# AbrahamSanders/realtime-codec-agent

Hardware: AMD Instinct MI355X
Metric: batch-encode audio-hours/hour (+ xRT and p50 frame-step latency of 1 duplex stream in `duplex`) (higher is better)
Workload: dtype f32; 1 GPU; batch MagiCodec-style encode, 16 kHz stereo, 0.1 s chunks / 2.0 s context, 256 windows per step (BASELINE configs[1]); codebook=131072x16

## Files before the change

### include/rca.h

```cpp
#ifndef RCA_H
#define RCA_H

#include <stdint.h>

#ifdef __cplusplus
extern "C" {
#endif

#define RCA_OK 0
#define RCA_ERR_ARG -1
#define RCA_ERR_HIP -2
#define RCA_ERR_STATE -3
#define RCA_ERR_MISSING -4

#define RCA_MAX_STAGES 8

typedef struct rca_codec rca_codec_t;
typedef struct rca_lm rca_lm_t;

#define RCA_F32 0
#define RCA_BF16 1
#define RCA_Q8_0 2
#define RCA_F16 3
#define RCA_Q6_K 5
// ... 70 lines not shown
                              float* pcm_dev, void* stream);
int rca_codec_decode_rows_dev(rca_codec_t* h, const int64_t* codes_dev, const int64_t* src_off_dev, int32_t B, int32_t F, int32_t n_samples,
                              float* pcm_dev, const int64_t* dst_off_dev, int64_t code_span, int64_t pcm_span, void* stream);
int rca_codec_decode_error(rca_codec_t* h, void* stream, int32_t* raised);

#define RCA_JOIN_HEAD 1
#define RCA_JOIN_TAIL 2
typedef struct {
    int64_t seg_off;
    int64_t n;
    int64_t out_off;
    int32_t flags;
    int32_t reserved;
} rca_join_seg_t;
int rca_codec_crossfade_join_dev(rca_codec_t* h, const float* seg_dev, int64_t seg_span, const rca_join_seg_t* segs_dev,
                                 const rca_join_seg_t* segs_host, int32_t n_segs, const float* fade_in_dev, int32_t n_fade, float* out_dev,
                                 int64_t out_span, void* stream);

int rca_codec_encode_tail(rca_codec_t* h, const float* pcm_host, int32_t B, int32_t T, int32_t n_keep, int64_t* codes_host);
int rca_codec_decode_tail(rca_codec_t* h, const int64_t* codes_host, int32_t B, int32_t F, int32_t n_samples, float* pcm_host);
int rca_codec_set_stream_graphs(rca_codec_t* h, int32_t enable);
int rca_codec_set_mfma_mode(rca_codec_t* h, int32_t mode);
int rca_codec_receptive_field(const rca_codec_t* h, int32_t* enc_left_frames, int32_t* dec_left_frames);
int rca_codec_set_window_trim(rca_codec_t* h, int32_t enable);

int rca_codec_decode(rca_codec_t* h, const int64_t* codes_host, int32_t B, int32_t F, float* pcm_host);
int rca_codec_decode_dev(rca_codec_t* h, const int64_t* codes_dev, int32_t B, int32_t F, float* pcm_dev,
                         void* stream);

int rca_codec_encoder_dev(rca_codec_t* h, const float* pcm_dev, int32_t B, int32_t T, float* ze_dev, void* stream);
int rca_codec_quantize_dev(rca_codec_t* h, const float* ze_dev, int64_t rows, int64_t* codes_dev, void* stream);
int rca_codec_decoder_dev(rca_codec_t* h, const float* zq_dev, int32_t B, int32_t F, float* pcm_dev, void* stream);
int rca_codec_codebook_dev(rca_codec_t* h, const float** out_dev);

int rca_codec_codebook(rca_codec_t* h, float* out_host);

int rca_codec_encode_tap(rca_codec_t* h, const float* pcm_host, int32_t B, int32_t T, int32_t layer,
                         float* out_host, int64_t out_numel);

int rca_codec_encode_tap_bf16(rca_codec_t* h, const float* pcm_host, int32_t B, int32_t T, int32_t layer,
                              uint16_t* hi_host, uint16_t* lo_host, int64_t numel);

int rca_codec_set_variant(rca_codec_t* h, int32_t variant);

int rca_codec_profile(rca_codec_t* h, int32_t enable);
int rca_codec_profile_read(rca_codec_t* h, int32_t kclass, double* total_ms, int64_t* launches, double* flops,
// ... 127 lines not shown
```

### realtime_codec_agent_amd/_native.py

```python
from __future__ import annotations

import ctypes as C
import os
import subprocess
from typing import Dict, Iterable, List, Optional, Tuple

import numpy as np

_PKG_DIR = os.path.dirname(os.path.abspath(__file__))
CSRC_DIR = os.path.join(_PKG_DIR, "csrc")
LIB_PATH = os.environ.get("RCA_LIB_PATH") or os.path.join(_PKG_DIR, "librca_hip.so")
HIP_SOURCES = ["rca_codec.hip", "rca_lm.hip"]
HIPCC_FLAGS = ["--offload-arch=gfx950", "-O3", "-ffp-contract=off", "-std=c++17", "-fPIC", "-shared",
               "-Wno-unused-result", "-mllvm", "-amdgpu-kernarg-preload-count=14"]

MAX_STAGES = 8
RCA_F32, RCA_BF16, RCA_Q8_0, RCA_F16, RCA_Q4_K, RCA_Q6_K, RCA_Q5_K, RCA_Q4_0, RCA_Q4_1 = 0, 1, 2, 3, 4, 5, 6, 7, 8


class RcaError(RuntimeError):
    pass


class Q8Blocks:
# ... 306 lines not shown
            if verbose:
                print(" ".join(cmd))
            subprocess.check_call(cmd)
            os.replace(LIB_PATH + sfx, LIB_PATH)
            with open(_stamp_path() + sfx, "w") as f:
                f.write(key + "\n")
            os.replace(_stamp_path() + sfx, _stamp_path())
        finally:
            for t in tmps + [_stamp_path() + sfx]:
                if os.path.exists(t):
                    os.remove(t)
    return LIB_PATH


_lib = None

ABI_SYMBOLS = [
    "rca_last_error", "rca_device_count", "rca_device_sync", "rca_version",
    "rca_codec_create", "rca_codec_destroy", "rca_codec_hop", "rca_codec_num_frames",
    "rca_codec_encode", "rca_codec_encode_dev", "rca_codec_encode_windows_dev", "rca_codec_encode_chunk_range_dev", "rca_codec_encode_rows_dev",
    "rca_codec_ingest_rows_dev", "rca_codec_ingest_supported",
    "rca_codec_decode_rows_dev", "rca_codec_decode_error", "rca_codec_crossfade_join_dev",
    "rca_codec_decode", "rca_codec_decode_dev",
    "rca_codec_encode_tail_dev", "rca_codec_decode_tail_dev", "rca_codec_encode_tail", "rca_codec_decode_tail", "rca_codec_set_stream_graphs", "rca_codec_receptive_field", "rca_codec_set_window_trim",
    "rca_codec_encoder_dev", "rca_codec_quantize_dev", "rca_codec_decoder_dev", "rca_codec_codebook_dev",
    "rca_codec_codebook", "rca_codec_encode_tap", "rca_codec_encode_tap_bf16", "rca_codec_set_variant", "rca_codec_sync",
    "rca_codec_profile", "rca_codec_profile_read",
    "rca_lm_create", "rca_lm_create_random", "rca_lm_destroy", "rca_lm_reset", "rca_lm_eval",
    "rca_lm_get_n_tokens", "rca_lm_set_n_tokens", "rca_lm_get_logits", "rca_lm_get_logits_row",
    "rca_lm_logits_dev", "rca_lm_sampler_init", "rca_lm_sample", "rca_lm_step", "rca_lm_token_probs",
    "rca_lm_sync", "rca_lm_set_graphs", "rca_lm_mask_head_rows", "rca_lm_set_mfma_prefill", "rca_lm_set_logits_all",
    "rca_lm_persist_codec_embeddings", "rca_lm_create_shared", "rca_lm_eval_async", "rca_lm_copy_kv", "rca_lm_swap_kv",
    "rca_lm_set_low_priority", "rca_lm_frame", "rca_lm_weight_format", "rca_lm_set_attn_fuse", "rca_lm_prefill_route",
    "rca_lm_set_act_format", "rca_lm_get_act_format", "rca_lm_gemv_tap", "rca_lm_kv_remove", "rca_lm_kv_read",
    "rca_lm_kv_write", "rca_lm_attn_tap", "rca_lm_score", "rca_lm_score_rows_tap",
    "rca_duplex_frame", "rca_codec_workspace_sig", "rca_codec_stream_handoff", "rca_codec_codebook_size", "rca_codec_set_mfma_mode", "rca_lm_step_probe", "rca_duplex_prepare", "rca_duplex_precapture",
    "rca_lm_group_create", "rca_lm_group_destroy", "rca_lm_group_step",
]


def lib():
    global _lib
    if _lib is not None:
        return _lib
    if not os.path.exists(LIB_PATH):
        raise RcaError(
            f"{LIB_PATH} not found: build the HIP extension first (python -c 'import __graft_entry__ as g; g.build()'). "
# ... 55 lines not shown
```

### realtime_codec_agent_amd/codec.py

```python
from __future__ import annotations

import ctypes as C
from typing import Dict, Optional, Tuple

import numpy as np

from . import _native as N
from .codec_model import CodecConfig, init_codec_weights


class HipCodec:
    def __init__(self, cfg: CodecConfig, weights: Dict[str, np.ndarray], device: int = 0):
        self.cfg = cfg
        self.device = device
        self._lib = N.lib()
        self._h = C.c_void_p()
        tensors, keep = N.make_tensors(weights)
        ccfg = N.codec_config_c(cfg)
        N.check(self._lib.rca_codec_create(C.byref(ccfg), tensors, len(weights), device, C.byref(self._h)), "rca_codec_create")
        del keep
        self.hop = cfg.hop
        self.mfma_mode = 0

    def close(self):
# ... 102 lines not shown
                                                    C.c_void_p(lo.ctypes.data if lo is not None else None), C.c_int64(B * Cn * L)),
                "rca_codec_encode_tap_bf16")
        unblock = lambda a: np.ascontiguousarray(a.transpose(0, 1, 3, 2).reshape(B, Cn, L))
        return unblock(hi), (unblock(lo) if lo is not None else None)

    def encode_dev(self, pcm_ptr: int, B: int, T: int, codes_ptr: int, stream: int = 0) -> None:
        N.check(self._lib.rca_codec_encode_dev(self._h, C.c_void_p(pcm_ptr), B, T, C.c_void_p(codes_ptr), C.c_void_p(stream)), "rca_codec_encode_dev")

    def decode_dev(self, codes_ptr: int, B: int, F: int, pcm_ptr: int, stream: int = 0) -> None:
        N.check(self._lib.rca_codec_decode_dev(self._h, C.c_void_p(codes_ptr), B, F, C.c_void_p(pcm_ptr), C.c_void_p(stream)), "rca_codec_decode_dev")

    def encode_tail_dev(self, pcm_ptr: int, B: int, T: int, n_keep: int, codes_ptr: int, stream: int = 0) -> None:
        N.check(self._lib.rca_codec_encode_tail_dev(self._h, C.c_void_p(pcm_ptr), B, T, n_keep, C.c_void_p(codes_ptr), C.c_void_p(stream)),
                "rca_codec_encode_tail_dev")

    def decode_tail_dev(self, codes_ptr: int, B: int, F: int, n_samples: int, pcm_ptr: int, stream: int = 0) -> None:
        N.check(self._lib.rca_codec_decode_tail_dev(self._h, C.c_void_p(codes_ptr), B, F, n_samples, C.c_void_p(pcm_ptr), C.c_void_p(stream)),
                "rca_codec_decode_tail_dev")

    def receptive_field(self) -> Tuple[int, int]:
        a, b = C.c_int32(), C.c_int32()
        N.check(self._lib.rca_codec_receptive_field(self._h, C.byref(a), C.byref(b)), "rca_codec_receptive_field")
        return a.value, b.value

    def set_window_trim(self, enable: bool) -> None:
        N.check(self._lib.rca_codec_set_window_trim(self._h, int(bool(enable))), "rca_codec_set_window_trim")

    def encode_windows_dev(self, audio_ptr: int, Cn: int, Nsamp: int, chunk: int, ctx: int, batch_windows: int, codes_ptr: int,
                           codes_per_channel: int, stream: int = 0) -> None:
        N.check(self._lib.rca_codec_encode_windows_dev(self._h, C.c_void_p(audio_ptr), Cn, C.c_int64(Nsamp), chunk, ctx, batch_windows,
                                                       C.c_void_p(codes_ptr), C.c_int64(codes_per_channel), C.c_void_p(stream)),
                "rca_codec_encode_windows_dev")

    def encode_chunk_range_dev(self, audio_ptr: int, Cn: int, Nsamp: int, chunk: int, ctx: int, batch_windows: int, chunk_begin: int,
                               chunk_end: int, codes_ptr: int, codes_per_channel: int, stream: int = 0) -> None:
        N.check(self._lib.rca_codec_encode_chunk_range_dev(self._h, C.c_void_p(audio_ptr), Cn, C.c_int64(Nsamp), chunk, ctx, batch_windows,
                                                           C.c_int64(chunk_begin), C.c_int64(chunk_end), C.c_void_p(codes_ptr),
                                                           C.c_int64(codes_per_channel), C.c_void_p(stream)),
                "rca_codec_encode_chunk_range_dev")

    def encode_rows_dev(self, audio_ptr: int, src_off_ptr: int, B: int, T: int, n_keep: int, codes_ptr: int, dst_off_ptr: int, span: int,
                        stream: int = 0) -> None:
        N.check(self._lib.rca_codec_encode_rows_dev(self._h, C.c_void_p(audio_ptr), C.c_void_p(src_off_ptr), B, T, n_keep, C.c_void_p(codes_ptr),
                                                    C.c_void_p(dst_off_ptr), C.c_int64(span), C.c_void_p(stream)), "rca_codec_encode_rows_dev")

    def ingest_supported(self, up: int, down: int, n_taps: int) -> bool:
# ... 261 lines not shown
```

### realtime_codec_agent_amd/csrc/rca_codec.hip

```cpp
#include <stdarg.h>

#include <algorithm>
#include <array>
#include <cmath>
#include <map>
#include <type_traits>

#include "rca_common.h"

namespace rca {
thread_local char g_err[512] = {0};
}
using namespace rca;

typedef float f32x16 __attribute__((ext_vector_type(16)));

#define RCA_LAT_MAX_FRAMES 64
#define RCA_LDS_BUDGET (152 * 1024)

typedef float f32x4 __attribute__((ext_vector_type(4)));

struct RowSrc {
    const float* base;
    int C;
// ... 184 lines not shown
#ifndef RCA_CONV_WPB
#define RCA_CONV_WPB 1
#endif
#ifndef RCA_CONV_OCC
#define RCA_CONV_OCC 2
#endif
#ifndef RCA_CONV_PIPE
#define RCA_CONV_PIPE 1
#endif
#ifndef RCA_CONV_PRIO
#define RCA_CONV_PRIO 1
#endif
#ifndef RCA_CONV_ABUF
#define RCA_CONV_ABUF 1
#endif
#ifndef RCA_CONV_EPRIO
#define RCA_CONV_EPRIO 1
#endif
#ifdef RCA_ABL_NOBREAD
#define RCA_ABL_BREAD(x) (slope)
#else
#define RCA_ABL_BREAD(x) (x)
#endif
typedef __bf16 conv_bf16x8 __attribute__((ext_vector_type(8)));
typedef __bf16 conv_bf16x2 __attribute__((ext_vector_type(2)));
__device__ __forceinline__ unsigned conv_pack_bf16x2(float a, float b) {
    const conv_bf16x2 v = {(__bf16)a, (__bf16)b};
    return __builtin_bit_cast(unsigned, v);
}
template <int BF>
__device__ __forceinline__ void conv_split8(const float (&w)[8], uint4& hi, uint4& lo) {
    unsigned ph[4], pl[4];
#pragma unroll
    for (int j = 0; j < 4; ++j) {
        ph[j] = conv_pack_bf16x2(w[2 * j], w[2 * j + 1]);
        pl[j] = BF == 3 ? conv_pack_bf16x2(w[2 * j] - __uint_as_float(ph[j] << 16), w[2 * j + 1] - __uint_as_float(ph[j] & 0xffff0000u)) : 0u;
    }
    hi = make_uint4(ph[0], ph[1], ph[2], ph[3]);
    lo = make_uint4(pl[0], pl[1], pl[2], pl[3]);
}
template <int KS, int S, int CIC, int WM, int WN, int FUSE, int TR, int BF = 0, int FULLC = 0>
__global__ __launch_bounds__(64 * RCA_CONV_WPB, (((KS == 8 && CIC == 2) || (KS == 16 && CIC == 1)) && WM * WN < 8) ? 3 : RCA_CONV_OCC) void conv1d_mfma_kernel(const float* __restrict__ x, const float* __restrict__ wp,
                                                          const float* __restrict__ bias, float* __restrict__ y,
                                                          int Cin, int Lin, int Cout, int Lout, long Ncols, int nchunks,
                                                          int pre, float slope, FuseIn fin, TrInfo tr) {
    constexpr int MT = WM * 32;
// ... 191 lines not shown
        for (int q = 0; q < 4; ++q) {
            const f32x4 bq = *reinterpret_cast<const f32x4*>(bias + co0 + wm * 32 + 8 * q + 4 * half);
#pragma unroll
            for (int j = 0; j < 4; ++j)
#pragma unroll
                for (int wn = 0; wn < WN; ++wn) acc[wm][wn][4 * q + j] = bq[j];
        }
    }

    auto stage_write_t = [&](int buf, auto act_tag) __attribute__((always_inline)) {
        constexpr bool ACT = decltype(act_tag)::value;
#ifdef RCA_ABL_NOWRITE
        return;
#endif
        float* dst = xs + buf * BUF;
#pragma unroll
        for (int cl = 0; cl < CIC; ++cl) {
#pragma unroll
            for (int r = 0; r < RE; ++r) {
                float v[PW];
#pragma unroll
                for (int j = 0; j < PW; ++j) {
                    v[j] = sreg[cl][r][j];
                    if (ACT && !FUSE) v[j] = fmaxf(v[j], v[j] * slope);
                }
                if (U > NW + 2 || 64 * PW * (r + 1) <= E || s_loff[r] >= 0) {
#pragma unroll
                    for (int j = 0; j < PW; ++j) dst[cl * S * U + s_loff[r] + j * U] = v[j];
                }
            }
        }
    };
    auto stage_write = [&](int buf) __attribute__((always_inline)) {
        if (pre & 1) stage_write_t(buf, std::true_type{});
        else stage_write_t(buf, std::false_type{});
    };

    auto compute_t = [&](int buf, int cn, auto edge_tag) __attribute__((always_inline)) {
        constexpr bool EDGE = decltype(edge_tag)::value;
        const float* xb = xs + buf * BUF;
        const float4* pn[WM];
#pragma unroll
        for (int wm = 0; wm < WM; ++wm) pn[wm] = w_ptr(wm, cn);
        constexpr int NB = (KPC * WN > 32) ? ((KPC % 4 == 0) ? 4 : 2) : (KPC * WN == 32 && WN == 4) ? 2 : 1;
        constexpr int PB = KPC / NB;
        static_assert(KPC % NB == 0, "batching");
#pragma unroll
// ... 184 lines not shown
    }

    if (RCA_CONV_EPRIO) __builtin_amdgcn_s_setprio(0);
    RCA_TL_STAMP(tl2);
    const long orow = TR ? tr.Lout : Lout;
    const bool full_rows = co0 + MT <= Cout;
    float* const yw = y + ((long)b_base * Cout + co0) * orow;
#pragma unroll
    for (int wn = 0; wn < WN; ++wn) {
        const int dn = 1 - lead + wn * 32 + (lane & 31);
        if (dn >= ncol_left) continue;
        int bb, t;
        rel_bt(dn, bb, t);
        int ocol = t;
        if (TR) {
            ocol = tr.s * t - tr.padL + phase;
            if (ocol < 0 || ocol >= (int)orow) continue;
        }
        const unsigned voff = ((unsigned)bb * (unsigned)(Cout * (int)orow) + (unsigned)ocol + (unsigned)(4 * half) * (unsigned)orow) * 4u;
        if (pre & 2) {
#pragma unroll
            for (int wm = 0; wm < WM; ++wm)
#pragma unroll
                for (int r = 0; r < 16; ++r) acc[wm][wn][r] = fmaxf(acc[wm][wn][r], acc[wm][wn][r] * slope);
        }
        if (full_rows) {
#pragma unroll
            for (int wm = 0; wm < WM; ++wm)
#pragma unroll
                for (int r = 0; r < 16; ++r) {
                    const int cu = wm * 32 + (r & 3) + 8 * (r >> 2);
                    char* const yr = reinterpret_cast<char*>(yw + (long)cu * orow);
                    *reinterpret_cast<float*>(yr + voff) = acc[wm][wn][r];
                }
        } else {
#pragma unroll
            for (int wm = 0; wm < WM; ++wm)
#pragma unroll
                for (int r = 0; r < 16; ++r) {
                    const int cu = wm * 32 + (r & 3) + 8 * (r >> 2);
                    char* const yr = reinterpret_cast<char*>(yw + (long)cu * orow);
                    if (co0 + cu + 4 * half < Cout) *reinterpret_cast<float*>(yr + voff) = acc[wm][wn][r];
                }
        }
    }
#ifdef RCA_CONV_TIMELINE
    if (tl_buf && lane == 0) {
        const long tl3 = (long)wall_clock64();
        const unsigned hw = __builtin_amdgcn_s_getreg((31 << 11) | (0 << 6) | 4);
        const unsigned xcc = __builtin_amdgcn_s_getreg((3 << 11) | (0 << 6) | 20);
        constexpr int region = KS == 4 ? 0 : KS == 8 ? 1 : KS == 10 ? 2 : KS == 16 ? 3 : KS == 3 ? 4 : 5;
        long* o = tl_buf + ((long)region * 65536 + ((blockIdx.x * RCA_CONV_WPB + wave) & 0xFFFF)) * 8;
        o[6] = tl_load | (tl_mfma << 32);
        o[7] = tl_write | ((long)nchunks << 32);
        o[0] = tl0; o[1] = tl1; o[2] = tl2; o[3] = tl3;
        o[4] = (long)hw | ((long)xcc << 32);
        o[5] = (long)KS | ((long)S << 8) | ((long)WM << 16) | ((long)wave << 24) | ((long)blockIdx.x << 32);
    }
#endif
}

template <int NWN, bool PRE>
__global__ __launch_bounds__(64, 2) void conv_first_mfma_kernel(const float* __restrict__ wp, const float* __restrict__ bias,
                                                               float* __restrict__ y, int Cout, int Lout, long Ncols, int post, float slope,
                                                               FuseIn fin) {
    constexpr int NW = NWN * 32;
    constexpr int E = (NW + 2) * 2;
    constexpr int NBLK = 2 * NWN + 1;
    constexpr int RS = 136;
    constexpr int ZERO = 128;
    constexpr int CIN = 32, KQ = CIN / 2;
    extern __shared__ __attribute__((aligned(16))) float ring[];
#ifdef RCA_CONV_TIMELINE
    long* const tl_buf = rca_prof_buf;
#endif
    RCA_TL_STAMP(tl0);
    const int lane = threadIdx.x & 63;
    const int half = lane >> 5, jl = lane & 31;
    const int n_co = Cout / 64;
    const long wg = blockIdx.x;
    const int xcd = (int)(wg & 7);
    const long seq = wg >> 3;
    const int co_tile = __builtin_amdgcn_readfirstlane((int)(seq % n_co));
    const long n0 = ((seq / n_co) * 8 + xcd) * NW;
    const int co0 = co_tile * 64;
    if (n0 >= Ncols) return;
    const long n_base = n0 > 0 ? n0 - 1 : 0;
    const int b_base = __builtin_amdgcn_readfirstlane((int)((unsigned)n_base / (unsigned)Lout));
    const int t_base = (int)(n_base - (long)b_base * Lout);
    const int lead = n0 > 0 ? 0 : 1;
    const long left = Ncols - n_base;
    const int ncol_left = left > NW + 2 ? NW + 2 : (int)left;
    auto rel_bt = [&](int dn, int& bb, int& tt) {
        int dt = dn + t_base;
        bb = dt >= Lout ? 1 : 0;
        tt = bb ? dt - Lout : dt;
    };

    const int ch_in = jl;
    float a_in[4];
#pragma unroll
    for (int m = 0; m < 4; ++m) a_in[m] = (2 * m + half < 7) ? fin.w_in[ch_in * 7 + 2 * m + half] : -0.0f;
    f32x16 b_in;
#pragma unroll
    for (int r = 0; r < 16; ++r) b_in[r] = fin.b_in[(r & 3) + 8 * (r >> 2) + 4 * half];
    long o0, o1;
    if (fin.src.row_off) {
// ... 10 lines not shown
    const long om = o0 < o1 ? o0 : o1;
    const rca_rsrc_t rs_pcm = rca_make_rsrc(fin.src.base + om, 0x7FFFFFFF);
    const unsigned prow0 = (unsigned)(o0 - om), prow1 = (unsigned)(o1 - om);
    constexpr unsigned OOB = 0x80000000u;
    auto pcm_load = [&](int bk, float (&pb)[4]) __attribute__((always_inline)) {
        const int e = 32 * bk + jl;
        const int dn = (e >> 1) - lead;
        const bool ok = e < E && dn >= 0 && dn < ncol_left;
        int bb, t;
        rel_bt(ok ? dn : 0, bb, t);
        const int i = 2 * t + (e & 1) - 3 + half;
        const unsigned ro = bb ? prow1 : prow0;
#pragma unroll
        for (int m = 0; m < 4; ++m) {
            const int j = i + 2 * m;
            const unsigned off = (ok && 2 * m + half < 7 && j >= 0 && j < fin.src.T) ? (ro + (unsigned)j) * 4u : OOB;
            pb[m] = rca_buffer_load_f32(rs_pcm, (int)off, 0, 0);
        }
    };
    auto cin_mfma = [&](int m, const float (&pb)[4], f32x16& d) __attribute__((always_inline)) {
        d = __builtin_amdgcn_mfma_f32_32x32x2f32(a_in[m], pb[m], m == 0 ? b_in : d, 0, 0, 0);
    };
    const int w_lane = 4 * half * RS + jl;
    auto cin_write = [&](int bk, f32x16& d, int r0, int r1) __attribute__((always_inline)) {
#pragma unroll
        for (int r = r0; r < r1; ++r) {
            float v = d[r];
            if (PRE) v = fmaxf(v, v * slope);
            ring[w_lane + ((r & 3) + 8 * (r >> 2)) * RS + ((32 * bk) & 127)] = v;
        }
    };

    if (lane < CIN) ring[lane * RS + ZERO] = 0.0f;
    float pa[4], pb[4];
    float4 a[2][KQ];
    {
        float p2[4];
        pcm_load(0, pa);
        pcm_load(1, pb);
        pcm_load(2, p2);
        __builtin_amdgcn_sched_barrier(0);
        const rca_rsrc_t rs_w = rca_make_rsrc(reinterpret_cast<const float4*>(wp) + (long)co_tile * 2 * KQ * 64, 0x7FFFFFFF);
#pragma unroll
        for (int wm = 0; wm < 2; ++wm)
#pragma unroll
            for (int q = 0; q < KQ; ++q) {
                const rca_f32x4_t v = rca_buffer_load_f32x4(rs_w, lane * 16, (wm * KQ + q) * 1024, 0);
                a[wm][q] = make_float4(v[0], v[1], v[2], v[3]);
            }
        __builtin_amdgcn_sched_barrier(0);
        f32x16 d0, d1;
#pragma unroll
        for (int m = 0; m < 4; ++m) { cin_mfma(m, pa, d0); cin_mfma(m, pb, d1); }
        cin_write(0, d0, 0, 16);
#pragma unroll
        for (int m = 0; m < 4; ++m) cin_mfma(m, p2, d0);
        cin_write(1, d1, 0, 16);
        cin_write(2, d0, 0, 16);
    }
    if (NBLK > 3) pcm_load(3, pa);
    if (NBLK > 4) pcm_load(4, pb);
    __builtin_amdgcn_wave_barrier();
    RCA_TL_STAMP(tl1);
#ifdef RCA_CONV_TIMELINE
    long tl_load = 1 << 30, tl_mfma = 0, tl_write = 0;
#endif

    const rca_rsrc_t rs_y = rca_make_rsrc(y + ((long)b_base * Cout + co0) * Lout, 0x7FFFFFFF);
    __builtin_amdgcn_s_setprio(RCA_CONV_EPRIO);
#pragma unroll
    for (int wn = 0; wn < NWN; ++wn) {
        RCA_TL_STAMP(ta);
        const int j = 32 * wn + jl;
        int bz, tz;
        rel_bt(1 - lead + j, bz, tz);
        const int ad0 = (half == 0 && tz == 0) ? ZERO : ((2 * j + 1 + half) & 127);
        const int ad1 = (half == 1 && tz == Lout - 1) ? ZERO : ((2 * j + 3 + half) & 127);
        f32x16 acc[2];
#pragma unroll
        for (int wm = 0; wm < 2; ++wm)
#pragma unroll
            for (int q = 0; q < 4; ++q) {
                const f32x4 bq = *reinterpret_cast<const f32x4*>(bias + co0 + wm * 32 + 8 * q + 4 * half);
#pragma unroll
                for (int jj = 0; jj < 4; ++jj) acc[wm][4 * q + jj] = bq[jj];
            }
        const bool more = 2 * wn + 4 < NBLK;
        f32x16 d;
        float bcur[4], bnxt[4];
        auto b_read = [&](int c, float (&bv)[4]) __attribute__((always_inline)) {
#pragma unroll
            for (int cl = 0; cl < 2; ++cl) {
                bv[2 * cl] = ring[ad0 + (2 * c + cl) * RS];
                bv[2 * cl + 1] = ring[ad1 + (2 * c + cl) * RS];
            }
        };
        b_read(0, bcur);
#pragma unroll
        for (int c = 0; c < KQ; ++c) {
            if (c + 1 < KQ) b_read(c + 1, bnxt);
#pragma unroll
            for (int kp = 0; kp < 4; ++kp) {
#pragma unroll
                for (int wm = 0; wm < 2; ++wm) {
                    const float4 q4 = a[wm][c];
                    const float av = kp == 0 ? q4.x : kp == 1 ? q4.y : kp == 2 ? q4.z : q4.w;
                    acc[wm] = __builtin_amdgcn_mfma_f32_32x32x2f32(av, bcur[kp], acc[wm], 0, 0, 0);
                }
                if (c == 0 && 2 * wn + 3 < NBLK) cin_mfma(kp, pa, d);
                if (c == 3 && more) cin_mfma(kp, pb, d);
            }
            if (c == 2 && 2 * wn + 3 < NBLK) cin_write(2 * wn + 3, d, 0, 16);
            if (more && c >= 4 && (c & 3) == 3) cin_write(2 * wn + 4, d, 4 * (c >> 2) - 4, 4 * (c >> 2));
            if (c == 1 && 2 * wn + 5 < NBLK) pcm_load(2 * wn + 5, pa);
            if (c == 4 && 2 * wn + 6 < NBLK) pcm_load(2 * wn + 6, pb);
            if (c + 1 < KQ) {
#pragma unroll
                for (int i = 0; i < 4; ++i) bcur[i] = bnxt[i];
            }
            __builtin_amdgcn_sched_barrier(0);
        }
        if (more) cin_write(2 * wn + 4, d, 12, 16);
        __builtin_amdgcn_wave_barrier();
        RCA_TL_STAMP(tb);
        const int dn = 1 - lead + j;
        int bb, t;
        rel_bt(dn, bb, t);
        const unsigned voff = dn < ncol_left ? ((unsigned)bb * (unsigned)(Cout * Lout) + (unsigned)t + (unsigned)(4 * half * Lout)) * 4u : OOB;
        if (post) {
#pragma unroll
            for (int wm = 0; wm < 2; ++wm)
#pragma unroll
                for (int r = 0; r < 16; ++r) acc[wm][r] = fmaxf(acc[wm][r], acc[wm][r] * slope);
        }
#pragma unroll
        for (int wm = 0; wm < 2; ++wm)
#pragma unroll
            for (int r = 0; r < 16; ++r) rca_buffer_store_f32(acc[wm][r], rs_y, (int)voff, (wm * 32 + (r & 3) + 8 * (r >> 2)) * Lout * 4, 0);
        RCA_TL_STAMP(tc);
        RCA_TL_MIN(tl_load, ta, tb); RCA_TL_ADD(tl_mfma, ta, tb); RCA_TL_ADD(tl_write, tb, tc);
    }
    if (RCA_CONV_EPRIO) __builtin_amdgcn_s_setprio(0);
    RCA_TL_STAMP(tl2);
#ifdef RCA_CONV_TIMELINE
    if (tl_buf && lane == 0) {
        const long tl3 = (long)wall_clock64();
        const unsigned hw = __builtin_amdgcn_s_getreg((31 << 11) | (0 << 6) | 4);
        const unsigned xcc = __builtin_amdgcn_s_getreg((3 << 11) | (0 << 6) | 20);
        long* o = tl_buf + ((long)blockIdx.x & 0xFFFF) * 8;
        o[6] = tl_load | (tl_mfma << 32);
        o[7] = tl_write | ((long)(2 * NWN) << 32);
        o[0] = tl0; o[1] = tl1; o[2] = tl2; o[3] = tl3;
        o[4] = (long)hw | ((long)xcc << 32);
        o[5] = 4L | (2L << 8) | (2L << 16) | ((long)blockIdx.x << 32);
    }
#endif
}

template <int KS, int S, int CIC, int FUSE>
__global__ __launch_bounds__(512) void conv1d_ws_kernel(const float* __restrict__ x, const float* __restrict__ wp,
                                                        const float* __restrict__ bias, float* __restrict__ y,
                                                        int Cin, int Lin, int Cout, int Lout, long Ncols, int nchunks,
                                                        int pre, float slope, FuseIn fin) {
    constexpr int WM = 2, WN = 2;
    constexpr int MT = WM * 32, NW = WN * 32;
    constexpr int U = ConvLds<S>::stride(NW);
    constexpr int KPC = CIC * KS / 2;
    constexpr int QPC = KPC / 4;
    constexpr int E = (NW + 2) * S;
    constexpr int RE = (E + 63) / 64;
    constexpr int padL = (KS - S + 1) / 2;
    constexpr int BUF = CIC * S * U + 4;
    constexpr int WBUF = WM * QPC * 64 * 4;
    static_assert(KPC % 4 == 0 && KPC <= 64, "chunk shape");
// ... 1369 lines not shown
    if (!h) return fail(RCA_ERR_ARG, "null");
    RCA_HIP(hipSetDevice(h->device));
    RCA_HIP(hipStreamSynchronize(h->stream));
    return RCA_OK;
}

template <int KS, int S, int CIC, int WM, int WN, int FUSE, int TR, int BF = 0>
static void launch_conv_cfg(const ConvLayer& L, const float* wp, int nchunks, const float* x, float* y, int Lin, int Lc, long Ncols,
                            float slope, const FuseIn& fin, const TrInfo& tr, hipStream_t st, int act) {
    constexpr int NT = RCA_CONV_WPB * WN * 32, MT = WM * 32;
    constexpr int lds = RCA_CONV_WPB * 2 * (CIC * S * ConvLds<S>::stride(WN * 32) + 4) * 4;
    static_assert(lds <= 65536, "LDS budget");
    const long col_tiles = (cdiv(Ncols, NT) + 7) / 8 * 8;
    dim3 grid((unsigned)(col_tiles * cdiv(L.cout, MT) * (TR ? tr.s : 1)));
    if constexpr (!FUSE && !TR && BF == 0) {
        if (L.cin % CIC == 0 && nchunks * CIC == L.cin) {
            conv1d_mfma_kernel<KS, S, CIC, WM, WN, 0, 0, 0, 1><<<grid, 64 * RCA_CONV_WPB, lds, st>>>(x, wp, L.bp, y, L.cin, Lin, L.cout, Lc, Ncols, nchunks, act, slope, fin, tr);
            return;
        }
    }
    conv1d_mfma_kernel<KS, S, CIC, WM, WN, FUSE, TR, BF><<<grid, 64 * RCA_CONV_WPB, lds, st>>>(x, wp, L.bp, y, L.cin, Lin, L.cout, Lc, Ncols, nchunks, act, slope, fin, tr);
}

template <int KS, int S, int CIC>
static int launch_conv_mfma(const ConvLayer& L, const float* x, float* y, int B, int Lin, int Lout, float slope, hipStream_t st,
                            const FuseIn* fuse = nullptr, int act = -1, int bf = 0) {
    if (act < 0) act = L.pre;
    const long Ncols = (long)B * Lout;
    if (bf) {
        const FuseIn none_b{};
        const TrInfo notr_b{};
        const bool big = (long)cdiv(Ncols, 64) * cdiv(L.cout, 64) >= 2048;
#define RCA_BF_LAUNCH(FU, BFM) do { \
            if (big) launch_conv_cfg<KS, S, CIC, 2, 2, FU, 0, BFM>(L, L.wp, L.nchunks, x, y, Lin, Lout, Ncols, slope, FU ? *fuse : none_b, notr_b, st, act); \
            else launch_conv_cfg<KS, S, CIC, 1, 1, FU, 0, BFM>(L, L.wp, L.nchunks, x, y, Lin, Lout, Ncols, slope, FU ? *fuse : none_b, notr_b, st, act); } while (0)
        if constexpr (KS == 4 || KS == 8 || KS == 16) {
            if (fuse) { if (bf == 3) RCA_BF_LAUNCH(1, 3); else RCA_BF_LAUNCH(1, 1); RCA_LAUNCH_CHECK(); return RCA_OK; }
        }
        if (fuse) return fail(RCA_ERR_ARG, "internal: fused first layer of this shape has no bf16 instantiation");
        if (bf == 3) RCA_BF_LAUNCH(0, 3); else RCA_BF_LAUNCH(0, 1);
#undef RCA_BF_LAUNCH
        RCA_LAUNCH_CHECK();
        return RCA_OK;
    }
    const long waves_big = (long)cdiv(Ncols, 64) * cdiv(L.cout, 64);
#ifdef RCA_CONV_FORCE_MID
    constexpr long BIG_MIN = 1L << 40, MID_MIN = 2048;
#else
    constexpr long BIG_MIN = 8192, MID_MIN = 2048;
#endif
    const FuseIn none{};
    const TrInfo notr{};
    if (fuse) {
        static const bool wide = []() { const char* e = getenv("RCA_FUSE_WIDE"); return !(e && e[0] == '0'); }();
        if constexpr (KS == 4 && S == 2) {
            const char* mi = getenv("RCA_FUSE_MFMA_IN");
            constexpr int NWN = 4;
            if (!(mi && mi[0] == '0') && wide && waves_big >= BIG_MIN && Lout >= NWN * 32 + 3 && L.cin == 32 && L.cout % 64 == 0) {
                const long col_tiles = (cdiv(Ncols, NWN * 32) + 7) / 8 * 8;
                const dim3 grid((unsigned)(col_tiles * (L.cout / 64)));
                constexpr int lds = 32 * 136 * 4;
                if (act & 1) conv_first_mfma_kernel<NWN, true><<<grid, 64, lds, st>>>(L.wp, L.bp, y, L.cout, Lout, Ncols, act & 2, slope, *fuse);
                else conv_first_mfma_kernel<NWN, false><<<grid, 64, lds, st>>>(L.wp, L.bp, y, L.cout, Lout, Ncols, act & 2, slope, *fuse);
                RCA_LAUNCH_CHECK();
                return RCA_OK;
            }
            if (wide && waves_big >= BIG_MIN && Lout >= 131 && L.cin % 2 == 0) {
                launch_conv_cfg<4, 2, 2, 2, 4, 1, 0>(L, L.wp, L.cin / 2, x, y, Lin, Lout, Ncols, slope, *fuse, notr, st, act);
                RCA_LAUNCH_CHECK();
                return RCA_OK;
            }
        }
        if (waves_big >= BIG_MIN) launch_conv_cfg<KS, S, CIC, 2, 2, 1, 0>(L, L.wp, L.nchunks, x, y, Lin, Lout, Ncols, slope, *fuse, notr, st, act);
        else launch_conv_cfg<KS, S, CIC, 1, 1, 1, 0>(L, L.wp, L.nchunks, x, y, Lin, Lout, Ncols, slope, *fuse, notr, st, act);
    } else {
        if (waves_big >= BIG_MIN) launch_conv_cfg<KS, S, CIC, 2, 2, 0, 0>(L, L.wp, L.nchunks, x, y, Lin, Lout, Ncols, slope, none, notr, st, act);
        else if (waves_big >= MID_MIN) launch_conv_cfg<KS, S, CIC, 1, 2, 0, 0>(L, L.wp, L.nchunks, x, y, Lin, Lout, Ncols, slope, none, notr, st, act);
        else if (KS == 3 && L.cout >= 64 && waves_big >= 1024) launch_conv_cfg<KS, S, CIC, (KS == 3 ? 2 : 1), 1, 0, 0>(L, L.wp, L.nchunks, x, y, Lin, Lout, Ncols, slope, none, notr, st, act);
        else launch_conv_cfg<KS, S, CIC, 1, 1, 0, 0>(L, L.wp, L.nchunks, x, y, Lin, Lout, Ncols, slope, none, notr, st, act);
    }
    RCA_LAUNCH_CHECK();
    return RCA_OK;
}

static int launch_convtr_mfma(const ConvLayer& L, const float* x, float* y, int B, int Lin, float slope, hipStream_t st) {
    const int Lc = Lin + 1;
// ... 282 lines not shown
                         esz * (double)Ly.cin * Ly.k * Ly.cout);
        const Bf16Pack& wp = h->bf16_packs[li];
        const conv_bf16raw *xh = hi_of(cur), *xl = lo_of(cur);
        conv_bf16raw *yh = hi_of(cur ^ 1), *yl = lo_of(cur ^ 1);
        float* yf = h->act[cur ^ 1].as<float>();
        if (!split && Ly.k == 10 && Ly.cout % 256 == 0) rc = launch_conv_bf16<10, 5, 4, 1, 0, 0, 2>(split, Ly, wp, xh, xl, yh, yl, yf, B, L, act, slope, st);
        else if (last) rc = launch_conv_bf16<3, 1, 4, 4, 1>(split, Ly, wp, xh, xl, yh, yl, yf, B, L, act, slope, st);
        else if (Ly.k == 4 && li == 1 && fuse_in)
            rc = launch_conv_bf16<4, 2, 2, 2, 0, 1>(split, Ly, wp, xh, xl, yh, yl, yf, B, L, act, slope, st, src, h->bf16_packs[0].w_in8, Ly.pre ? 1 : 0);
        else if (Ly.k == 4) rc = launch_conv_bf16<4, 2, 2, 2, 0>(split, Ly, wp, xh, xl, yh, yl, yf, B, L, act, slope, st);
        else if (Ly.k == 8) rc = launch_conv_bf16<8, 4, 4, 1, 0>(split, Ly, wp, xh, xl, yh, yl, yf, B, L, act, slope, st);
        else if (Ly.k == 10) rc = launch_conv_bf16<10, 5, 4, 1, 0>(split, Ly, wp, xh, xl, yh, yl, yf, B, L, act, slope, st);
        else rc = launch_conv_bf16<16, 8, 4, 1, 0>(split, Ly, wp, xh, xl, yh, yl, yf, B, L, act, slope, st);
        if (rc != RCA_OK) return rc;
        L = Lout;
        cur ^= 1;
        if (last && tap_layer == (int)li) RCA_HIP(hipMemcpyAsync(tap_dev, yf, (size_t)B * Ly.cout * L * 4, hipMemcpyDeviceToDevice, st));
        if (stop_at((int)li)) return RCA_OK;
    }
    *ze_out = h->act[cur].as<float>();
    return RCA_OK;
}

static int run_encoder(rca_codec* h, RowSrc src, int B, hipStream_t st, float** ze_out, int* F_out, int tap_layer, float* tap_dev,
                       int bf16_tap = -1, const conv_bf16raw** bf16_planes = nullptr, int keep = 0, int* Fz_out = nullptr) {
    const rca_codec_config_t& c = h->cfg;
    const int F = (src.T + h->hop - 1) / h->hop;
    const int Tp = F * h->hop;
    if (F < 1) return fail(RCA_ERR_ARG, "empty audio (T=%d)", src.T);
    if (Fz_out) *Fz_out = F;
    size_t max_elems = 0;
    {
        long L = Tp;
        max_elems = std::max(max_elems, (size_t)B * c.channels[0] * L);
        for (int i = 0; i < c.n_stages; ++i) { L /= c.strides[i]; max_elems = std::max(max_elems, (size_t)B * c.channels[i + 1] * L); }
        max_elems = std::max(max_elems, (size_t)B * c.latent_dim * L);
    }
    int rc;
    if ((rc = h->act[0].ensure(max_elems * 4)) != RCA_OK) return rc;
    if ((rc = h->act[1].ensure(max_elems * 4)) != RCA_OK) return rc;
    if (bf16_blk_ok(h, tap_layer) && (double)B * max_elems < 4.0e18 && Tp / h->enc[1].s >= 64) {
        *F_out = F;
        return run_encoder_bf16(h, src, B, Tp, max_elems, st, ze_out, tap_layer, tap_dev, bf16_tap, bf16_planes);
    }
    if (bf16_tap >= 0) return fail(RCA_ERR_ARG, "bf16 tap: encode() does not take the blocked bf16 pipeline here (mfma mode %d, B=%d T=%d)", h->mfma_mode, B, src.T);
    int cur = 0;
    int L = Tp;
    size_t first = 1;
    const ConvLayer& E0 = h->enc[0];
    const ConvLayer& E1 = h->enc[1];
    const bool fuse01 = !h->lat_mode && h->variant >= 1 && tap_layer != 0 && E0.k == 7 && E1.wp && E1.k == 2 * E1.s && (double)B * E1.cin * L < 4.0e9 &&
                        ((E1.k == 4 && E1.s == 2) || (E1.k == 8 && E1.s == 4) || (E1.k == 16 && E1.s == 8)) && L / E1.s >= 67 &&
                        (double)E1.cout * (L / E1.s) < 2.6e8 &&
                        (src.row_off ? (double)src.span : (double)src.C * (double)std::labs(src.chan_stride) + (double)std::labs(src.win_stride) + src.T) < 5.0e8;
    bool prev_post = false;
    auto handoff = [&](size_t next, int Lnext) {
        return tap_layer < 0 && h->variant == 1 && !h->lat_mode && next < h->enc.size() && h->enc[next].pre && mfma_conv_ok(h, h->enc[next], B, Lnext, 0);
    };
    if (fuse01) {
        float* y = h->act[cur].as<float>();
        FuseIn fin{src, E0.w, E0.b};
        const float slope = c.leaky_slope;
        const int Lout = L / E1.s;
        {
            ProfScope ps(h, st, 0, 2.0 * E1.cin * E1.k * E1.cout * (double)B * Lout + 2.0 * E0.k * E0.cout * (double)B * L,
                         4.0 * ((double)B * src.T + (double)B * E1.cout * Lout + (double)E1.cin * E1.k * E1.cout));
            prev_post = handoff(2, Lout);
            const int act = (E1.pre ? 1 : 0) | (prev_post ? 2 : 0);
            if (h->variant == 2 && try_conv_ws(E1, nullptr, y, B, L, Lout, slope, st, &fin)) { rc = RCA_OK; RCA_LAUNCH_CHECK(); }
            else if (E1.k == 4) rc = launch_conv_mfma<4, 2, 4>(E1, nullptr, y, B, L, Lout, slope, st, &fin, act, h->mfma_mode);
            else if (E1.k == 8) rc = launch_conv_mfma<8, 4, RCA_CIC_K8>(E1, nullptr, y, B, L, Lout, slope, st, &fin, act, h->mfma_mode);
            else rc = launch_conv_mfma<16, 8, RCA_CIC_K16>(E1, nullptr, y, B, L, Lout, slope, st, &fin, act, h->mfma_mode);
        }
        if (rc != RCA_OK) return rc;
        L = Lout;
        first = 2;
// ... 102 lines not shown
    RowDst dst{codes, B, (long)F, 0, F};
    return run_quantize(h, ze, 0, B, F, 0, F, dst, st, nullptr);
}

static int trimmable_frames(const rca_codec* h, int F, int keep) { return std::max(0, F - keep - h->enc_left_frames); }

extern "C" int rca_codec_encode_tail_dev(rca_codec_t* h, const float* pcm, int32_t B, int32_t T, int32_t n_keep, int64_t* codes,
                                         void* stream) {
    if (!h || !pcm || !codes || B < 1 || T < 1 || n_keep < 1) return fail(RCA_ERR_ARG, "encode_tail: bad argument (B=%d T=%d keep=%d)", B, T, n_keep);
    const int F = (T + h->hop - 1) / h->hop;
    if (n_keep > F) return fail(RCA_ERR_ARG, "encode_tail: %d frames wanted, the window holds %d", n_keep, F);
    RCA_HIP(hipSetDevice(h->device));
    hipStream_t st = pick_stream(h, stream);
    const int j = trimmable_frames(h, F, n_keep);
    RowSrc src{pcm + (long)j * h->hop, B, (long)T, 0, T - j * h->hop};
    float* ze; int Ft, rc;
    h->lat_mode = h->variant >= 1 && (long)B * (F - j) <= RCA_LAT_MAX_FRAMES;
    int Fz;
    rc = run_encoder(h, src, B, st, &ze, &Ft, -1, nullptr, -1, nullptr, n_keep, &Fz);
    h->lat_mode = false;
    if (rc != RCA_OK) return rc;
    RowDst dst{codes, B, (long)n_keep, 0, n_keep};
    return run_quantize(h, ze, 0, B, Fz, Fz - n_keep, n_keep, dst, st, nullptr);
}

extern "C" int rca_codec_receptive_field(const rca_codec_t* h, int32_t* enc_left_frames, int32_t* dec_left_frames) {
    if (!h || !enc_left_frames || !dec_left_frames) return fail(RCA_ERR_ARG, "null");
    *enc_left_frames = h->enc_left_frames;
    *dec_left_frames = h->dec_left_frames;
    return RCA_OK;
}

extern "C" int rca_codec_set_window_trim(rca_codec_t* h, int32_t enable) {
    if (!h) return fail(RCA_ERR_ARG, "null");
    h->window_trim = enable != 0;
    return RCA_OK;
}

extern "C" int rca_codec_encode(rca_codec_t* h, const float* pcm_host, int32_t B, int32_t T, int64_t* codes_host) {
    if (!h || !pcm_host || !codes_host || B < 1 || T < 1) return fail(RCA_ERR_ARG, "encode: bad argument (B=%d T=%d)", B, T);
    RCA_HIP(hipSetDevice(h->device));
    const int F = (T + h->hop - 1) / h->hop;
    int rc;
    if ((rc = h->io_a.ensure((size_t)B * T * 4)) != RCA_OK) return rc;
    if ((rc = h->io_b.ensure((size_t)B * F * 8)) != RCA_OK) return rc;
    RCA_HIP(hipMemcpyAsync(h->io_a.p, pcm_host, (size_t)B * T * 4, hipMemcpyHostToDevice, h->stream));
// ... 634 lines not shown
```

Baseline: 3496 audio-hours/hour.

## Choose first-layer fused conv column width per shape, with runtime group count

The fused first conv MFMA kernel used to process a fixed 4 groups of 32 columns per wave. It can now take a runtime group count picked by a cost model over slots, so each wave covers more columns and amortizes the ring prologue and epilogue. The loop is restructured into even and odd parity groups so ring offsets stay compile-time. Leaky ReLU now uses an inline v_max_f32 asm helper, and a plan-query API is added. The risks are fewer waves, which lowers occupancy and parallelism, and weaker unrolling in the runtime-count path.

```diff
diff --git a/include/rca.h b/include/rca.h
--- a/include/rca.h
+++ b/include/rca.h
@@ -116,6 +116,7 @@
 int rca_codec_set_stream_graphs(rca_codec_t* h, int32_t enable);
 int rca_codec_set_mfma_mode(rca_codec_t* h, int32_t mode);
 int rca_codec_receptive_field(const rca_codec_t* h, int32_t* enc_left_frames, int32_t* dec_left_frames);
+int rca_codec_first_layer_plan(const rca_codec_t* h, int32_t B, int32_t T, int32_t* cols_per_wave);
 int rca_codec_set_window_trim(rca_codec_t* h, int32_t enable);
 
 int rca_codec_decode(rca_codec_t* h, const int64_t* codes_host, int32_t B, int32_t F, float* pcm_host);
diff --git a/realtime_codec_agent_amd/_native.py b/realtime_codec_agent_amd/_native.py
--- a/realtime_codec_agent_amd/_native.py
+++ b/realtime_codec_agent_amd/_native.py
@@ -352,7 +352,7 @@
     "rca_codec_ingest_rows_dev", "rca_codec_ingest_supported",
     "rca_codec_decode_rows_dev", "rca_codec_decode_error", "rca_codec_crossfade_join_dev",
     "rca_codec_decode", "rca_codec_decode_dev",
-    "rca_codec_encode_tail_dev", "rca_codec_decode_tail_dev", "rca_codec_encode_tail", "rca_codec_decode_tail", "rca_codec_set_stream_graphs", "rca_codec_receptive_field", "rca_codec_set_window_trim",
+    "rca_codec_encode_tail_dev", "rca_codec_decode_tail_dev", "rca_codec_encode_tail", "rca_codec_decode_tail", "rca_codec_set_stream_graphs", "rca_codec_receptive_field", "rca_codec_first_layer_plan", "rca_codec_set_window_trim",
     "rca_codec_encoder_dev", "rca_codec_quantize_dev", "rca_codec_decoder_dev", "rca_codec_codebook_dev",
     "rca_codec_codebook", "rca_codec_encode_tap", "rca_codec_encode_tap_bf16", "rca_codec_set_variant", "rca_codec_sync",
     "rca_codec_profile", "rca_codec_profile_read",
diff --git a/realtime_codec_agent_amd/codec.py b/realtime_codec_agent_amd/codec.py
--- a/realtime_codec_agent_amd/codec.py
+++ b/realtime_codec_agent_amd/codec.py
@@ -148,6 +148,11 @@
         a, b = C.c_int32(), C.c_int32()
         N.check(self._lib.rca_codec_receptive_field(self._h, C.byref(a), C.byref(b)), "rca_codec_receptive_field")
         return a.value, b.value
+
+    def first_layer_plan(self, B: int, T: int) -> int:
+        n = C.c_int32()
+        N.check(self._lib.rca_codec_first_layer_plan(self._h, int(B), int(T), C.byref(n)), "rca_codec_first_layer_plan")
+        return n.value
 
     def set_window_trim(self, enable: bool) -> None:
         N.check(self._lib.rca_codec_set_window_trim(self._h, int(bool(enable))), "rca_codec_set_window_trim")
diff --git a/realtime_codec_agent_amd/csrc/rca_codec.hip b/realtime_codec_agent_amd/csrc/rca_codec.hip
--- a/realtime_codec_agent_amd/csrc/rca_codec.hip
+++ b/realtime_codec_agent_amd/csrc/rca_codec.hip
@@ -230,6 +230,12 @@
 #else
 #define RCA_ABL_BREAD(x) (x)
 #endif
+__device__ __forceinline__ float conv_lrelu(float v, float slope) {
+    const float m = v * slope;
+    float r;
+    asm("v_max_f32 %0, %1, %2" : "=v"(r) : "v"(v), "v"(m));
+    return r;
+}
 typedef __bf16 conv_bf16x8 __attribute__((ext_vector_type(8)));
 typedef __bf16 conv_bf16x2 __attribute__((ext_vector_type(2)));
 __device__ __forceinline__ unsigned conv_pack_bf16x2(float a, float b) {
@@ -467,7 +473,7 @@
 #pragma unroll
                 for (int j = 0; j < PW; ++j) {
                     v[j] = sreg[cl][r][j];
-                    if (ACT && !FUSE) v[j] = fmaxf(v[j], v[j] * slope);
+                    if (ACT && !FUSE) v[j] = conv_lrelu(v[j], slope);
                 }
                 if (U > NW + 2 || 64 * PW * (r + 1) <= E || s_loff[r] >= 0) {
 #pragma unroll
@@ -698,7 +704,7 @@
 #pragma unroll
             for (int wm = 0; wm < WM; ++wm)
 #pragma unroll
-                for (int r = 0; r < 16; ++r) acc[wm][wn][r] = fmaxf(acc[wm][wn][r], acc[wm][wn][r] * slope);
+                for (int r = 0; r < 16; ++r) acc[wm][wn][r] = conv_lrelu(acc[wm][wn][r], slope);
         }
         if (full_rows) {
 #pragma unroll
@@ -739,10 +745,11 @@
 template <int NWN, bool PRE>
 __global__ __launch_bounds__(64, 2) void conv_first_mfma_kernel(const float* __restrict__ wp, const float* __restrict__ bias,
                                                                float* __restrict__ y, int Cout, int Lout, long Ncols, int post, float slope,
-                                                               FuseIn fin) {
-    constexpr int NW = NWN * 32;
-    constexpr int E = (NW + 2) * 2;
-    constexpr int NBLK = 2 * NWN + 1;
+                                                               FuseIn fin, int ngroups) {
+    static_assert(NWN % 2 == 0, "a wave walks whole ring periods");
+    const int ng = NWN ? NWN : ngroups;
+    const int NW = ng * 32;
+    const int E = (NW + 2) * 2;
     constexpr int RS = 136;
     constexpr int ZERO = 128;
     constexpr int CIN = 32, KQ = CIN / 2;
@@ -758,7 +765,7 @@
     const int xcd = (int)(wg & 7);
     const long seq = wg >> 3;
     const int co_tile = __builtin_amdgcn_readfirstlane((int)(seq % n_co));
-    const long n0 = ((seq / n_co) * 8 + xcd) * NW;
+    const long n0 = ((seq / n_co) * 8 + xcd) * (long)NW;
     const int co0 = co_tile * 64;
     if (n0 >= Ncols) return;
     const long n_base = n0 > 0 ? n0 - 1 : 0;
@@ -815,12 +822,12 @@
         d = __builtin_amdgcn_mfma_f32_32x32x2f32(a_in[m], pb[m], m == 0 ? b_in : d, 0, 0, 0);
     };
     const int w_lane = 4 * half * RS + jl;
-    auto cin_write = [&](int bk, f32x16& d, int r0, int r1) __attribute__((always_inline)) {
+    auto cin_write = [&](int rb, f32x16& d, int r0, int r1) __attribute__((always_inline)) {
 #pragma unroll
         for (int r = r0; r < r1; ++r) {
             float v = d[r];
-            if (PRE) v = fmaxf(v, v * slope);
-            ring[w_lane + ((r & 3) + 8 * (r >> 2)) * RS + ((32 * bk) & 127)] = v;
+            if (PRE) v = conv_lrelu(v, slope);
+            ring[w_lane + ((r & 3) + 8 * (r >> 2)) * RS + rb] = v;
         }
     };
 
@@ -848,11 +855,11 @@
         cin_write(0, d0, 0, 16);
 #pragma unroll
         for (int m = 0; m < 4; ++m) cin_mfma(m, p2, d0);
-        cin_write(1, d1, 0, 16);
-        cin_write(2, d0, 0, 16);
-    }
-    if (NBLK > 3) pcm_load(3, pa);
-    if (NBLK > 4) pcm_load(4, pb);
+        cin_write(32, d1, 0, 16);
+        cin_write(64, d0, 0, 16);
+    }
+    pcm_load(3, pa);
+    pcm_load(4, pb);
     __builtin_amdgcn_wave_barrier();
     RCA_TL_STAMP(tl1);
 #ifdef RCA_CONV_TIMELINE
@@ -861,24 +868,26 @@
 
     const rca_rsrc_t rs_y = rca_make_rsrc(y + ((long)b_base * Cout + co0) * Lout, 0x7FFFFFFF);
     __builtin_amdgcn_s_setprio(RCA_CONV_EPRIO);
-#pragma unroll
-    for (int wn = 0; wn < NWN; ++wn) {
+    auto group = [&](auto par_tag, auto cin_tag, auto pcm_tag, int wn) __attribute__((always_inline)) {
+        constexpr int PAR = decltype(par_tag)::value;
+        constexpr bool CIN = decltype(cin_tag)::value, PCM = decltype(pcm_tag)::value;
         RCA_TL_STAMP(ta);
         const int j = 32 * wn + jl;
         int bz, tz;
         rel_bt(1 - lead + j, bz, tz);
-        const int ad0 = (half == 0 && tz == 0) ? ZERO : ((2 * j + 1 + half) & 127);
-        const int ad1 = (half == 1 && tz == Lout - 1) ? ZERO : ((2 * j + 3 + half) & 127);
+        const int ad0 = (half == 0 && tz == 0) ? ZERO : ((64 * PAR + 2 * jl + 1 + half) & 127);
+        const int ad1 = (half == 1 && tz == Lout - 1) ? ZERO : ((64 * PAR + 2 * jl + 3 + half) & 127);
         f32x16 acc[2];
+        int bias_o = co0;
+        if (NWN == 0) asm volatile("" : "+s"(bias_o));
 #pragma unroll
         for (int wm = 0; wm < 2; ++wm)
 #pragma unroll
             for (int q = 0; q < 4; ++q) {
-                const f32x4 bq = *reinterpret_cast<const f32x4*>(bias + co0 + wm * 32 + 8 * q + 4 * half);
+                const f32x4 bq = *reinterpret_cast<const f32x4*>(bias + bias_o + wm * 32 + 8 * q + 4 * half);
 #pragma unroll
                 for (int jj = 0; jj < 4; ++jj) acc[wm][4 * q + jj] = bq[jj];
             }
-        const bool more = 2 * wn + 4 < NBLK;
         f32x16 d;
         float bcur[4], bnxt[4];
         auto b_read = [&](int c, float (&bv)[4]) __attribute__((always_inline)) {
@@ -900,20 +909,20 @@
                     const float av = kp == 0 ? q4.x : kp == 1 ? q4.y : kp == 2 ? q4.z : q4.w;
                     acc[wm] = __builtin_amdgcn_mfma_f32_32x32x2f32(av, bcur[kp], acc[wm], 0, 0, 0);
                 }
-                if (c == 0 && 2 * wn + 3 < NBLK) cin_mfma(kp, pa, d);
-                if (c == 3 && more) cin_mfma(kp, pb, d);
-            }
-            if (c == 2 && 2 * wn + 3 < NBLK) cin_write(2 * wn + 3, d, 0, 16);
-            if (more && c >= 4 && (c & 3) == 3) cin_write(2 * wn + 4, d, 4 * (c >> 2) - 4, 4 * (c >> 2));
-            if (c == 1 && 2 * wn + 5 < NBLK) pcm_load(2 * wn + 5, pa);
-            if (c == 4 && 2 * wn + 6 < NBLK) pcm_load(2 * wn + 6, pb);
+                if (c == 0 && CIN) cin_mfma(kp, pa, d);
+                if (c == 3 && CIN) cin_mfma(kp, pb, d);
+            }
+            if (c == 2 && CIN) cin_write((64 * PAR + 96) & 127, d, 0, 16);
+            if (CIN && c >= 4 && (c & 3) == 3) cin_write(64 * PAR, d, 4 * (c >> 2) - 4, 4 * (c >> 2));
+            if (c == 1 && PCM) pcm_load(2 * wn + 5, pa);
+            if (c == 4 && PCM) pcm_load(2 * wn + 6, pb);
             if (c + 1 < KQ) {
 #pragma unroll
                 for (int i = 0; i < 4; ++i) bcur[i] = bnxt[i];
             }
             __builtin_amdgcn_sched_barrier(0);
         }
-        if (more) cin_write(2 * wn + 4, d, 12, 16);
+        if (CIN) cin_write(64 * PAR, d, 12, 16);
         __builtin_amdgcn_wave_barrier();
         RCA_TL_STAMP(tb);
         const int dn = 1 - lead + j;
@@ -924,7 +933,7 @@
 #pragma unroll
             for (int wm = 0; wm < 2; ++wm)
 #pragma unroll
-                for (int r = 0; r < 16; ++r) acc[wm][r] = fmaxf(acc[wm][r], acc[wm][r] * slope);
+                for (int r = 0; r < 16; ++r) acc[wm][r] = conv_lrelu(acc[wm][r], slope);
         }
 #pragma unroll
         for (int wm = 0; wm < 2; ++wm)
@@ -932,7 +941,17 @@
             for (int r = 0; r < 16; ++r) rca_buffer_store_f32(acc[wm][r], rs_y, (int)voff, (wm * 32 + (r & 3) + 8 * (r >> 2)) * Lout * 4, 0);
         RCA_TL_STAMP(tc);
         RCA_TL_MIN(tl_load, ta, tb); RCA_TL_ADD(tl_mfma, ta, tb); RCA_TL_ADD(tl_write, tb, tc);
-    }
+    };
+    constexpr std::integral_constant<int, 0> even{};
+    constexpr std::integral_constant<int, 1> odd{};
+    constexpr int UNROLL = NWN ? NWN / 2 : 1;
+#pragma unroll UNROLL
+    for (int wn = 0; wn < ng - 2; wn += 2) {
+        group(even, std::true_type{}, std::true_type{}, wn);
+        group(odd, std::true_type{}, std::true_type{}, wn + 1);
+    }
+    group(even, std::true_type{}, std::false_type{}, ng - 2);
+    group(odd, std::false_type{}, std::false_type{}, ng - 1);
     if (RCA_CONV_EPRIO) __builtin_amdgcn_s_setprio(0);
     RCA_TL_STAMP(tl2);
 #ifdef RCA_CONV_TIMELINE
@@ -942,7 +961,7 @@
         const unsigned xcc = __builtin_amdgcn_s_getreg((3 << 11) | (0 << 6) | 20);
         long* o = tl_buf + ((long)blockIdx.x & 0xFFFF) * 8;
         o[6] = tl_load | (tl_mfma << 32);
-        o[7] = tl_write | ((long)(2 * NWN) << 32);
+        o[7] = tl_write | ((long)(2 * ng) << 32);
         o[0] = tl0; o[1] = tl1; o[2] = tl2; o[3] = tl3;
         o[4] = (long)hw | ((long)xcc << 32);
         o[5] = 4L | (2L << 8) | (2L << 16) | ((long)blockIdx.x << 32);
@@ -2358,6 +2377,27 @@
     conv1d_mfma_kernel<KS, S, CIC, WM, WN, FUSE, TR, BF><<<grid, 64 * RCA_CONV_WPB, lds, st>>>(x, wp, L.bp, y, L.cin, Lin, L.cout, Lc, Ncols, nchunks, act, slope, fin, tr);
 }
 
+#ifdef RCA_CONV_FORCE_MID
+constexpr long CONV_BIG_MIN = 1L << 40, CONV_MID_MIN = 2048;
+#else
+constexpr long CONV_BIG_MIN = 8192, CONV_MID_MIN = 2048;
+#endif
+
+static int first_layer_groups(const ConvLayer& L, long Ncols, int Lout) {
+    static const bool wide = []() { const char* e = getenv("RCA_FUSE_WIDE"); return !(e && e[0] == '0'); }();
+    const char* mi = getenv("RCA_FUSE_MFMA_IN");
+    if ((mi && mi[0] == '0') || !wide || cdiv(Ncols, 64) * cdiv(L.cout, 64) < CONV_BIG_MIN || Lout < 4 * 32 + 3 || L.cin != 32 || L.cout % 64) return 0;
+    constexpr long SLOTS = 2048;
+    const int nmax = std::min(128, ((Lout - 3) / 32) & ~1);
+    int best = 4;
+    long best_cost = 0;
+    for (int n = 8; n <= nmax; n += 2) {
+        const long cost = cdiv(cdiv(Ncols, 32L * n), SLOTS) * (n + 2);
+        if (!best_cost || cost <= best_cost) { best = n; best_cost = cost; }
+    }
+    return best;
+}
+
 template <int KS, int S, int CIC>
 static int launch_conv_mfma(const ConvLayer& L, const float* x, float* y, int B, int Lin, int Lout, float slope, hipStream_t st,
                             const FuseIn* fuse = nullptr, int act = -1, int bf = 0) {
@@ -2380,24 +2420,20 @@
         return RCA_OK;
     }
     const long waves_big = (long)cdiv(Ncols, 64) * cdiv(L.cout, 64);
-#ifdef RCA_CONV_FORCE_MID
-    constexpr long BIG_MIN = 1L << 40, MID_MIN = 2048;
-#else
-    constexpr long BIG_MIN = 8192, MID_MIN = 2048;
-#endif
+    constexpr long BIG_MIN = CONV_BIG_MIN, MID_MIN = CONV_MID_MIN;
     const FuseIn none{};
     const TrInfo notr{};
     if (fuse) {
         static const bool wide = []() { const char* e = getenv("RCA_FUSE_WIDE"); return !(e && e[0] == '0'); }();
         if constexpr (KS == 4 && S == 2) {
-            const char* mi = getenv("RCA_FUSE_MFMA_IN");
-            constexpr int NWN = 4;
-            if (!(mi && mi[0] == '0') && wide && waves_big >= BIG_MIN && Lout >= NWN * 32 + 3 && L.cin == 32 && L.cout % 64 == 0) {
-                const long col_tiles = (cdiv(Ncols, NWN * 32) + 7) / 8 * 8;
+            if (const int ng = first_layer_groups(L, Ncols, Lout)) {
+                const long col_tiles = (cdiv(Ncols, 32L * ng) + 7) / 8 * 8;
                 const dim3 grid((unsigned)(col_tiles * (L.cout / 64)));
                 constexpr int lds = 32 * 136 * 4;
-                if (act & 1) conv_first_mfma_kernel<NWN, true><<<grid, 64, lds, st>>>(L.wp, L.bp, y, L.cout, Lout, Ncols, act & 2, slope, *fuse);
-                else conv_first_mfma_kernel<NWN, false><<<grid, 64, lds, st>>>(L.wp, L.bp, y, L.cout, Lout, Ncols, act & 2, slope, *fuse);
+#define RCA_FIRST_LAUNCH(NWN, PRE) conv_first_mfma_kernel<NWN, PRE><<<grid, 64, lds, st>>>(L.wp, L.bp, y, L.cout, Lout, Ncols, act & 2, slope, *fuse, ng)
+                if (ng == 4) { if (act & 1) RCA_FIRST_LAUNCH(4, true); else RCA_FIRST_LAUNCH(4, false); }
+                else { if (act & 1) RCA_FIRST_LAUNCH(0, true); else RCA_FIRST_LAUNCH(0, false); }
+#undef RCA_FIRST_LAUNCH
                 RCA_LAUNCH_CHECK();
                 return RCA_OK;
             }
@@ -2726,6 +2762,14 @@
     return RCA_OK;
 }
 
+static bool fuse01_shape_ok(const rca_codec* h, int B, int L) {
+    const ConvLayer& E0 = h->enc[0];
+    const ConvLayer& E1 = h->enc[1];
+    return !h->lat_mode && h->variant >= 1 && E0.k == 7 && E1.wp && E1.k == 2 * E1.s && (double)B * E1.cin * L < 4.0e9 &&
+           ((E1.k == 4 && E1.s == 2) || (E1.k == 8 && E1.s == 4) || (E1.k == 16 && E1.s == 8)) && L / E1.s >= 67 &&
+           (double)E1.cout * (L / E1.s) < 2.6e8;
+}
+
 static int run_encoder(rca_codec* h, RowSrc src, int B, hipStream_t st, float** ze_out, int* F_out, int tap_layer, float* tap_dev,
                        int bf16_tap = -1, const conv_bf16raw** bf16_planes = nullptr, int keep = 0, int* Fz_out = nullptr) {
     const rca_codec_config_t& c = h->cfg;
@@ -2753,9 +2797,7 @@
     size_t first = 1;
     const ConvLayer& E0 = h->enc[0];
     const ConvLayer& E1 = h->enc[1];
-    const bool fuse01 = !h->lat_mode && h->variant >= 1 && tap_layer != 0 && E0.k == 7 && E1.wp && E1.k == 2 * E1.s && (double)B * E1.cin * L < 4.0e9 &&
-                        ((E1.k == 4 && E1.s == 2) || (E1.k == 8 && E1.s == 4) || (E1.k == 16 && E1.s == 8)) && L / E1.s >= 67 &&
-                        (double)E1.cout * (L / E1.s) < 2.6e8 &&
+    const bool fuse01 = fuse01_shape_ok(h, B, L) && tap_layer != 0 &&
                         (src.row_off ? (double)src.span : (double)src.C * (double)std::labs(src.chan_stride) + (double)std::labs(src.win_stride) + src.T) < 5.0e8;
     bool prev_post = false;
     auto handoff = [&](size_t next, int Lnext) {
@@ -2904,6 +2946,16 @@
     if (rc != RCA_OK) return rc;
     RowDst dst{codes, B, (long)n_keep, 0, n_keep};
     return run_quantize(h, ze, 0, B, Fz, Fz - n_keep, n_keep, dst, st, nullptr);
+}
+
+extern "C" int rca_codec_first_layer_plan(const rca_codec_t* h, int32_t B, int32_t T, int32_t* cols_per_wave) {
+    if (!h || !cols_per_wave || B < 1 || T < 1) return fail(RCA_ERR_ARG, "bad argument");
+    const int L = (T + h->hop - 1) / h->hop * h->hop;
+    *cols_per_wave = 0;
+    if (h->enc.size() < 2 || h->mfma_mode || h->variant != 1 || !fuse01_shape_ok(h, B, L)) return RCA_OK;
+    const ConvLayer& E1 = h->enc[1];
+    if (E1.k == 4 && E1.s == 2) *cols_per_wave = 32 * first_layer_groups(E1, (long)B * (L / E1.s), L / E1.s);
+    return RCA_OK;
 }
 
 extern "C" int rca_codec_receptive_field(const rca_codec_t* h, int32_t* enc_left_frames, int32_t* dec_left_frames) {
```

New measurement: 3515 audio-hours/hour, median of 6. About the same (+0.5%).
